# drprojects/superpoint_transformer

Hardware: AMD Instinct MI355X
Metric: Mpoints/s SPT fwd+bwd on S3DIS-scale NAG (higher is better)
Workload: dtype f32 (the reference's shipped matmul class - configs/train.yaml:60-61 `float32_matmul_precision: high` = TF32 / bf16x3 next to `precision: 32` - as bf16x3: matrix products on the bf16 pipe with split operands, attention and the backward of the fused layers and of the attention blocks' Linears hi*hi +

## Files before the change

include/spt_hip.h:

```cpp
#ifndef SPT_HIP_H
#define SPT_HIP_H

#include <stddef.h>
#include <stdint.h>

#ifdef __cplusplus
extern "C" {
#endif

typedef void* spt_stream_t;

enum spt_reduce_op {
  SPT_SUM = 0,
  SPT_MEAN = 1,
  SPT_MIN = 2,
  SPT_MAX = 3
};

typedef struct spt_gn_fwd_tables {
  const float* weight;
  const float* mean_scale;
  float eps;
  float* mean;
  float* rstd;
  float* am;
  float* scale;
} spt_gn_fwd_tables;
typedef struct spt_gn_bwd_tables {
  const float* weight;
  const float* mean_scale;
  const float* mean;
  const float* rstd;
  float* c1;
  float* c2;
  float* c3;
  float* gweight;
  float* gbias;
  float* gmean_scale;
} spt_gn_bwd_tables;

int spt_version(void);
const char* spt_last_error(void);

size_t spt_csr_build_workspace_bytes(int64_t n, int64_t num_seg);
int spt_csr_build(const int64_t* idx, int64_t n, int64_t num_seg,
                  int32_t* perm, int32_t* rowptr,
                  void* ws, size_t ws_bytes, spt_stream_t stream);
int spt_csr_pos_seg(const int32_t* rowptr, int64_t num_seg, int64_t n, int32_t* pos_seg,
                    spt_stream_t stream);
int spt_csr_gather_i64_i32(const int64_t* src, const int32_t* perm, int64_t n, int32_t* out,
                           spt_stream_t stream);

int spt_segcsr_reduce_f32(int op, const float* x, const int32_t* perm,
                          const int32_t* rowptr, int64_t n, int64_t num_seg,
                          int c, float* out, int32_t* arg, spt_stream_t stream);
int spt_segcsr_use_stream(int on);
int spt_segcsr_reduce_ex_f32(int op, const float* x, const int32_t* perm,
                             const int32_t* rowptr, int64_t n, int64_t num_seg,
                             int c, float* out, int32_t* arg, int formulation,
                             spt_stream_t stream);
int spt_segcsr_max_affine_ex_f32(const float* x, const int32_t* perm, const int32_t* rowptr,
                                 int64_t n, int64_t num_seg, int c, const float* am,
                                 const float* scale, const float* bias, float act_slope,
                                 const int64_t* seg_graph, float* out, int32_t* arg,
                                 int formulation, spt_stream_t stream);

int spt_segcsr_max_affine_f32(const float* x, const int32_t* perm, const int32_t* rowptr,
                              int64_t n, int64_t num_seg, int c, const float* am,
                              const float* scale, const float* bias, float act_slope,
                              const int64_t* seg_graph, float* out, int32_t* arg,
                              spt_stream_t stream);
int spt_segcsr_max_affine_bf16_supported(int c, int64_t n);
int spt_segcsr_max_affine_bf16(const void* x_bf16, const int32_t* perm, const int32_t* rowptr,
                               int64_t n, int64_t num_seg, int c, const float* am,
                               const float* scale, const float* bias, float act_slope,
                               const int64_t* seg_graph, float* out, int32_t* arg,
                               spt_stream_t stream);
int spt_segcsr_max_affine_raw_supported(int c, int64_t n);
int spt_segcsr_max_affine_raw_f32(const void* x, int x_is_bf16, const int32_t* perm,
                                  const int32_t* rowptr, int64_t n, int64_t num_seg, int c,
                                  const float* am, const float* scale, const float* bias,
                                  float act_slope, const int64_t* seg_graph, float* out,
                                  int32_t* arg, float* raw, spt_stream_t stream);
int spt_segcsr_reduce_bwd_f32(int op, const float* gout, const int32_t* arg,
                              const int64_t* idx, const int32_t* perm,
                              const int32_t* rowptr, int64_t n, int64_t num_seg,
                              int c, float* gx, spt_stream_t stream);


int spt_segcsr_sum_i64(const int64_t* x, const int32_t* perm,
                       const int32_t* rowptr, int64_t n, int64_t num_seg,
                       int c, int64_t* out, spt_stream_t stream);

int spt_gather_rows_f32(const float* x, const int64_t* idx, int64_t n,
                        int64_t num_src, int c, float* out, spt_stream_t stream);

int spt_unit_sphere_norm_f32(const float* pos, const int64_t* idx,
                             const int32_t* perm, const int32_t* rowptr,
                             const float* w_f32, const int64_t* w_i64,
                             int64_t n, int64_t num_seg, float* pos_out,
                             float* diam, float* center, spt_stream_t stream);
int spt_unit_sphere_assemble_f32(const float* pos, const int64_t* idx,
                                 const int32_t* perm, const int32_t* rowptr,
                                 const float* w_f32, const int64_t* w_i64,
                                 int64_t n, int64_t num_seg, const float* x, int cx,
                                 float* xcat, float* diam, float* center, spt_stream_t stream);
size_t spt_unit_sphere_workspace_bytes(int64_t n, int64_t num_seg);
int spt_unit_sphere_norm_ws_f32(const float* pos, const int64_t* idx, const int32_t* perm,
                                const int32_t* rowptr, const float* w_f32, const int64_t* w_i64,
                                int64_t n, int64_t num_seg, float* pos_out, float* diam,
                                float* center, void* ws, size_t ws_bytes, spt_stream_t stream);
int spt_unit_sphere_assemble_ws_f32(const float* pos, const int64_t* idx, const int32_t* perm,
                                    const int32_t* rowptr, const float* w_f32, const int64_t* w_i64,
                                    int64_t n, int64_t num_seg, const float* x, int cx, float* xcat,
                                    float* diam, float* center, void* ws, size_t ws_bytes,
                                    spt_stream_t stream);

size_t spt_graphnorm_workspace_bytes(int64_t r, int d, int num_graphs);
int spt_graphnorm_fwd_f32(const float* x, const int64_t* batch, int64_t r, int d,
                          int num_graphs, const float* weight, const float* bias,
                          const float* mean_scale, float eps, float act_slope,
                          float* y, float* mean, float* rstd, void* ws,
                          size_t ws_bytes, spt_stream_t stream);
int spt_graphnorm_bwd_f32(const float* x, const float* gy, const int64_t* batch,
                          int64_t r, int d, int num_graphs, const float* weight,
                          const float* bias, const float* mean_scale,
                          const float* mean, const float* rstd, float act_slope,
                          float* gx, float* gweight, float* gbias,
                          float* gmean_scale, void* ws, size_t ws_bytes,
                          spt_stream_t stream);
int spt_graphnorm_stats_f32(const float* x, const int64_t* batch, int64_t r, int d, int num_graphs,
                            const float* weight, const float* mean_scale, float eps, float* mean,
                            float* rstd, float* am, float* scale, void* ws, size_t ws_bytes,
                            spt_stream_t stream);
// ... 676 lines not shown
```

superpoint_transformer_amd/_lib.py:

```python
import ctypes
import os

import torch

_HERE = os.path.dirname(os.path.abspath(__file__))
LIB_PATH = os.path.join(_HERE, "lib", "libspt_hip.so")

_c = ctypes
_i64 = _c.c_int64
_int = _c.c_int
_p = _c.c_void_p
_sz = _c.c_size_t
_f32 = _c.c_float
_f64 = _c.c_double

SIGNATURES = {
    "spt_version": (_int, []),
    "spt_last_error": (_c.c_char_p, []),
    "spt_csr_build_workspace_bytes": (_sz, [_i64, _i64]),
    "spt_csr_build": (_int, [_p, _i64, _i64, _p, _p, _p, _sz, _p]),
    "spt_csr_pos_seg": (_int, [_p, _i64, _i64, _p, _p]),
    "spt_csr_gather_i64_i32": (_int, [_p, _p, _i64, _p, _p]),
    "spt_segcsr_reduce_f32": (_int, [_int, _p, _p, _p, _i64, _i64, _int, _p, _p, _p]),
    "spt_segcsr_max_affine_f32": (_int, [_p, _p, _p, _i64, _i64, _int, _p, _p, _p, _f32, _p, _p, _p, _p]),
    "spt_segcsr_max_affine_bf16_supported": (_int, [_int, _i64]),
    "spt_segcsr_max_affine_bf16": (_int, [_p, _p, _p, _i64, _i64, _int, _p, _p, _p, _f32, _p, _p, _p, _p]),
    "spt_segcsr_max_affine_raw_supported": (_int, [_int, _i64]),
    "spt_segcsr_max_affine_raw_f32": (_int, [_p, _int, _p, _p, _i64, _i64, _int, _p, _p, _p, _f32, _p, _p, _p,
                                             _p, _p]),
    "spt_graphnorm_bwd_stats_sparse_raw_f32": (_int, [_p, _p, _p, _p, _p, _i64, _i64, _int, _int, _p, _p, _p,
                                                      _f32, _p, _p, _sz, _p]),
    "spt_fused_linear_storage_supported": (_int, [_int, _int]),
    "spt_graphnorm_bwd_stats_sparse_ex_f32": (_int, [_p, _int, _p, _p, _p, _p, _i64, _i64, _int, _int, _p, _p,
                                                     _p, _f32, _p, _p, _sz, _p]),
    "spt_segcsr_reduce_bwd_f32": (_int, [_int, _p, _p, _p, _p, _p, _i64, _i64, _int, _p, _p]),
    "spt_segcsr_sum_i64": (_int, [_p, _p, _p, _i64, _i64, _int, _p, _p]),
    "spt_gather_rows_f32": (_int, [_p, _p, _i64, _i64, _int, _p, _p]),
    "spt_graphnorm_workspace_bytes": (_sz, [_i64, _int, _int]),
    "spt_graphnorm_fwd_f32": (_int, [_p, _p, _i64, _int, _int, _p, _p, _p, _f32, _f32,
                                     _p, _p, _p, _p, _sz, _p]),
    "spt_graphnorm_bwd_f32": (_int, [_p, _p, _p, _i64, _int, _int, _p, _p, _p, _p, _p,
                                     _f32, _p, _p, _p, _p, _p, _sz, _p]),
    "spt_graphnorm_stats_f32": (_int, [_p, _p, _i64, _int, _int, _p, _p, _f32, _p, _p, _p, _p,
                                       _p, _sz, _p]),
    "spt_graphnorm_bwd_acc_f32": (_int, [_p, _p, _p, _i64, _int, _int, _p, _p, _p, _p, _p,
                                         _f32, _p, _p, _p, _p, _p, _p, _sz, _p]),
    "spt_edge_attn_fwd_f32": (_int, [_p, _i64, _int, _int, _int, _p, _p, _p, _i64, _p, _int,
                                     _p, _p, _p, _p, _p, _p, _int, _f32, _p, _p, _p, _p]),
    "spt_edge_attn_bwd_workspace_bytes": (_sz, [_int, _int, _int, _int]),
    "spt_attn_use_mfma": (_int, [_int]),
    "spt_attn_bwd_packed": (_int, [_int]),
    "spt_attn_bwd_el_full_line": (_int, [_int]),
    "spt_attn_bwd_el_target_order": (_int, [_int]),
    "spt_attn_tile_record_ints": (_int, []),
    "spt_attn_pack_tile_ids_ex": (_int, [_p, _p, _p, _p, _i64, _p, _p]),
    "spt_attn_tile_record_ints_m": (_int, [_int]),
    "spt_attn_pack_tile_ids_m": (_int, [_p, _p, _p, _p, _i64, _int, _p, _p]),
    "spt_attn_mirror_prepare": (_int, [_p, _p, _i64, _i64, _p, _p, _p]),
    "spt_attn_pack_tile_ids_mirror": (_int, [_p, _p, _p, _p, _i64, _i64, _p, _p]),
    "spt_attn_split_pack_f32": (_int, [_p, _i64, _int, _int, _p, _p]),
    "spt_attn_split_grad_f32": (_int, [_p, _i64, _int, _int, _p, _p]),
    "spt_edge_attn_bwd_f32": (_int, [_p, _i64, _int, _int, _int, _p, _p, _p, _i64, _p, _int,
                                     _p, _p, _p, _p, _p, _p, _int, _f32, _p, _p, _p, _p,
                                     _p, _p, _p, _p, _p, _p, _p, _p, _p, _sz, _p]),
    "spt_edge_attn_bwd_acc_f32": (_int, [_p, _i64, _int, _int, _int, _p, _p, _p, _i64, _p, _int,
                                         _p, _p, _p, _p, _p, _p, _int, _f32, _p, _p, _p, _p,
                                         _p, _p, _int, _p, _p, _p, _p, _p, _p, _p, _sz, _p]),
    "spt_edge_attn_fwd_ex_f32": (_int, [_p, _i64, _int, _int, _int, _p, _p, _p, _i64, _p, _int,
                                        _p, _p, _p, _p, _p, _p, _int, _f32, _p, _p, _p, _int, _p]),
    "spt_attn_resolve_mode": (_int, [_int]),
    "spt_edge_attn_bwd_route": (_int, [_i64, _i64, _int, _int, _int, _int, _int, _int, _sz]),
    "spt_edge_attn_bwd_ex_workspace_bytes": (_sz, [_i64, _i64, _int, _int, _int, _int]),
    "spt_edge_attn_bwd_el_supported": (_int, [_int, _int, _int, _int, _int]),
    "spt_attn_pack_tile_ids": (_int, [_p, _p, _p, _i64, _p, _p]),
    "spt_edge_attn_bwd_ex_f32": (_int, [_p, _i64, _int, _int, _int, _p, _p, _p, _p, _p, _p, _p, _i64, _p, _int,
                                        _p, _p, _p, _p, _p, _p, _int, _f32, _p, _p, _p, _p,
                                        _p, _p, _int, _p, _p, _p, _p, _p, _p, _int, _p, _sz, _p]),
    "spt_grid_knn_workspace_bytes": (_sz, [_i64, _i64]),
    "spt_knn_use_cell_path": (_int, [_int]),
    "spt_segcsr_use_stream": (_int, [_int]),
    "spt_segcsr_reduce_ex_f32": (_int, [_int, _p, _p, _p, _i64, _i64, _int, _p, _p, _int, _p]),
    "spt_segcsr_max_affine_ex_f32": (_int, [_p, _p, _p, _i64, _i64, _int, _p, _p, _p, _f32, _p, _p, _p,
                                            _int, _p]),
    "spt_grid_knn_ex_f32": (_int, [_p, _i64, _p, _i64, _int, _f32, _f32, _p, _p, _int, _int, _int,
                                   _p, _p, _p, _int, _p, _sz, _p]),
    "spt_grid_knn_geof_f32": (_int, [_p, _i64, _int, _f32, _f32, _p, _p, _int, _int, _int, _int,
                                     _p, _p, _p, _p, _int, _p, _sz, _p]),
    "spt_grid_knn_after_f32": (_int, [_p, _i64, _p, _i64, _int, _f32, _f32, _p, _p, _int, _int, _p, _p,
                                      _p, _p, _p, _sz, _p]),
    "spt_grid_knn_f32": (_int, [_p, _i64, _p, _i64, _int, _f32, _f32, _p, _p, _int, _int, _int,
                                _p, _p, _p, _p, _sz, _p]),
    "spt_point_geof_dense_f32": (_int, [_p, _i64, _p, _int, _int, _int, _int, _p, _p, _p]),
    "spt_point_geof_dense_ld_f32": (_int, [_p, _i64, _p, _int, _i64, _int, _int, _int, _p, _p, _p]),
    "spt_bbox_f32": (_int, [_p, _i64, _p, _p]),
    "spt_knn_subsample_f32": (_int, [_p, _i64, _p, _f32, _int, _p, _p, _p]),
    "spt_grid_cell_ids_f32": (_int, [_p, _i64, _f32, _p, _p, _p, _p]),
    "spt_grid_count_cells_workspace_bytes": (_sz, [_i64]),
    "spt_grid_count_cells_f32": (_int, [_p, _i64, _f32, _p, _p, _p, _p, _sz, _p]),
    "spt_spatial_order_workspace_bytes": (_sz, [_i64, _i64]),
    "spt_spatial_order": (_int, [_p, _i64, _f32, _p, _p, _p, _p, _sz, _p]),
    "spt_point_geof_csr_f32": (_int, [_p, _i64, _p, _p, _int, _int, _int, _p, _p]),
    "spt_vertical_edge_features_f32": (_int, [_p, _i64] + [_p] * 13 + [_p]),
    "spt_edge_affinity_features_f32": (_int, [_p, _i64, _int, _p, _p, _i64, _p, _p]),
    "spt_edge_affinity_features_bwd_f32": (_int, [_p, _p, _i64, _int, _p, _p, _i64, _p, _p]),
    "spt_scatter_pca_f32": (_int, [_p, _p, _p, _i64, _p, _p, _p]),
# ... 271 lines not shown
```

superpoint_transformer_amd/csr.py:

```python
import weakref

import torch

from . import _lib

_ATTR = "_spt_csr_memo"
_ATTR_BAD = "_spt_csr_rejected"


class SegmentCSR:

    __slots__ = ("idx", "perm", "rowptr", "n", "num_seg", "_pos_seg")

    def __init__(self, idx, perm, rowptr, n, num_seg):
        self.idx = idx
        self.perm = perm
        self.rowptr = rowptr
        self.n = n
        self.num_seg = num_seg
        self._pos_seg = None

    def pos_seg(self):
        if self._pos_seg is None:
            out = torch.empty(max(self.n, 1), dtype=torch.int32, device=self.perm.device)
            with torch.cuda.device(out.device):
                st = _lib.lib.spt_csr_pos_seg(_lib.ptr(self.rowptr), self.num_seg, self.n,
                                              _lib.ptr(out), _lib.stream_ptr(out.device))
            _lib.check(st, "spt_csr_pos_seg")
            self._pos_seg = out[:self.n]
        return self._pos_seg

    def counts(self):
        return (self.rowptr[1:] - self.rowptr[:-1])


def build_csr(idx, num_seg):
    _lib.require_cuda(idx)
    if idx.dim() != 1:
        raise ValueError("segment index must be 1-D")
    idx = _lib.dense(idx, torch.int64, 8)
    n = idx.numel()
    num_seg = int(num_seg)
    if num_seg < 1:
        num_seg = 1
    dev = idx.device
    perm = torch.empty(max(n, 1), dtype=torch.int32, device=dev)
    rowptr = torch.empty(num_seg + 1, dtype=torch.int32, device=dev)
    ws_bytes = _lib.lib.spt_csr_build_workspace_bytes(n, num_seg)
    ws = torch.empty(max(ws_bytes, 1), dtype=torch.uint8, device=dev)
    with torch.cuda.device(dev):
        st = _lib.lib.spt_csr_build(
            _lib.ptr(idx), n, num_seg, _lib.ptr(perm), _lib.ptr(rowptr),
            _lib.ptr(ws), ws_bytes, _lib.stream_ptr(dev))
    _lib.check(st, "spt_csr_build")
    return SegmentCSR(idx.detach(), perm[:n], rowptr, n, num_seg)


def csr_of(idx, num_seg=None):
    if isinstance(idx, SegmentCSR):
        return idx
    if num_seg is None:
        num_seg = int(idx.max().item()) + 1 if idx.numel() > 0 else 1
    num_seg = max(int(num_seg), 1)
    memo = getattr(idx, _ATTR, None)
    key = (idx._version, num_seg, idx.data_ptr(), idx.numel())
    if memo is not None and key in memo:
        return memo[key]
    csr = build_csr(idx, num_seg)
    if memo is None or any(k[0] != idx._version for k in memo):
        memo = {}
        try:
            setattr(idx, _ATTR, memo)
        except Exception:
            return csr
    memo[key] = csr
    return csr


_USE_SUB_VIEWS = True
_USE_MIRROR = True


def use_mirror_views(on=True):
    global _USE_MIRROR
    old, _USE_MIRROR = _USE_MIRROR, bool(on)
    return old


def use_sub_views(on=True):
    global _USE_SUB_VIEWS
    old, _USE_SUB_VIEWS = _USE_SUB_VIEWS, bool(on)
    return old


class StaleCSRError(RuntimeError):
    """A stored ``sub`` adopted as the CSR view of a ``super_index`` turned out not to describe it."""


_PENDING = []
_CHECK_BITS = {1: "pointers do not run 0 .. n monotonically", 2: "a point id outside [0, n)",
               4: "membership: idx[points[j]] is not the cluster holding position j",
               8: "the points of a cluster are not in ascending order"}
_ORDER_ONLY = 8
_PINNED = {}


def _flag_text(v):
    return "; ".join(t for b, t in _CHECK_BITS.items() if v & b) or "ok"


def _pinned_slot():
    ring = _PINNED.get("ring")
    if ring is None:
        ring = _PINNED["ring"] = torch.zeros(256, dtype=torch.int32).pin_memory()
        _PINNED["next"] = 0
    busy = {h.data_ptr() for ev, h, *_ in _PENDING if ev is not None}
    for _ in range(ring.numel()):
        i = _PINNED["next"]
        _PINNED["next"] = (i + 1) % ring.numel()
        slot = ring[i:i + 1]
        if slot.data_ptr() not in busy:
            return slot
    return torch.zeros(1, dtype=torch.int32).pin_memory()


_MIRROR_BITS = {1: "a pair (i, i + M) that is not (s, t) / (t, s)", 2: "a self loop with s != t"}
MIRROR_ATTR = "_spt_mirror_pairs"


def _drop_view(ref, key, vkey, remember):
    idx = ref() if ref is not None else None
    if idx is None:
        return
    memo = getattr(idx, _ATTR, None)
    if memo is not None:
        memo.pop(key, None)
    if remember:
        try:
            setattr(idx, _ATTR_BAD, vkey)
        except Exception:
            pass


def verify_adopted(block=False):
    keep, failed = [], None
    for item in _PENDING:
        ev, host, what, ref, key, vkey = item
        if ev is None:
            if not block:
                keep.append(item)
                continue
            v = int(host.item())
        else:
            if block:
                ev.synchronize()
            if not ev.query():
                keep.append(item)
                continue
            v = int(host[0])
        if v and key == "mirror":
            ei = ref() if ref is not None else None
            if ei is not None:
                for a in (MIRROR_ATTR, _ATTR):
# ... 8 lines not shown
        if v:
            _drop_view(ref, key, vkey, remember=True)
        if v & ~_ORDER_ONLY and failed is None:
            failed = (what, v, None)
    _PENDING[:] = keep
    if failed is not None and failed[2] is not None:
        raise StaleCSRError(
            f"{failed[0]} was declared [i<j | j>i | loops] with mirrored halves ({MIRROR_ATTR}) but is not "
            f"({failed[2]}): the attention backward of that batch paired wrong edges - drop the attribute "
            "or rebuild the edge list (the hint has been removed: later batches sort by target)")
    if failed is not None:
        raise StaleCSRError(
            f"the stored CSR adopted as the view of {failed[0]} does not describe it "
            f"({_flag_text(failed[1])}): the segment kernels grouped wrong rows since that batch (inside "
            "their buffers: the adopted view is clamped) - rebuild the NAG's `sub` or call "
            "csr.use_sub_views(False)")


def adopt_csr(idx, num_seg, pointers, points, ascending=None, verify="now"):
    if not _USE_SUB_VIEWS or idx is None or ascending is False:
        return None
    n = idx.numel()
    num_seg = max(int(num_seg), 1)
    if (points.numel() != n or pointers.numel() != num_seg + 1
            or points.device != idx.device or pointers.device != idx.device):
        return None
    if idx.dtype != torch.int64 or not idx.is_contiguous() or idx.dim() != 1:
        return None
    _lib.require_cuda(idx)
    capturing = torch.cuda.is_current_stream_capturing()
    if _PENDING and not capturing:
        verify_adopted()
    memo = getattr(idx, _ATTR, None)
    key = (idx._version, num_seg, idx.data_ptr(), n)
    if memo is not None and key in memo:
        return memo[key]
    bad = getattr(idx, _ATTR_BAD, None)
    vkey = key + (points.data_ptr(), points._version, pointers.data_ptr(), pointers._version)
    if bad == vkey:
        return None
    dev = idx.device
    pl, ql = _lib.dense(points, torch.int64, 8), _lib.dense(pointers, torch.int64, 8)
    flag = torch.zeros(1, dtype=torch.int32, device=dev)
    perm = torch.empty(max(n, 1), dtype=torch.int32, device=dev)
    rowptr = torch.empty(num_seg + 1, dtype=torch.int32, device=dev)
    with torch.cuda.device(dev):
        st = _lib.lib.spt_csr_adopt_i64(_lib.ptr(idx), _lib.ptr(pl), _lib.ptr(ql), n, num_seg,
                                        _lib.ptr(perm), _lib.ptr(rowptr), _lib.ptr(flag),
                                        _lib.stream_ptr(dev))
    _lib.check(st, "spt_csr_adopt_i64")
    what = f"an index of {n} rows / {num_seg} segments"
    try:
        ref = weakref.ref(idx)
    except TypeError:
        ref = None
    if verify == "deferred" and capturing:
        _PENDING.append((None, flag, what, ref, key, vkey))
    elif verify == "deferred":
        host = _pinned_slot()
        host.copy_(flag, non_blocking=True)
        ev = torch.cuda.Event()
        ev.record(torch.cuda.current_stream(dev))
        _PENDING.append((ev, host, what, ref, key, vkey))
    elif int(flag.item()):
        try:
            setattr(idx, _ATTR_BAD, vkey)
        except Exception:
            pass
        return None
    csr = SegmentCSR(idx.detach(), perm[:n], rowptr, n, num_seg)
    if memo is None or any(k[0] != idx._version for k in memo):
        memo = {}
        try:
            setattr(idx, _ATTR, memo)
        except Exception:
            return csr
    memo[key] = csr
    return csr


class EdgeCSR:

    __slots__ = ("erowptr", "eperm", "tgt_sorted", "n", "e", "_view", "_src_sorted", "_tview",
                 "_tile_ids", "_ei", "_mirror", "_ei_ref")

    def __init__(self, erowptr, eperm, tgt_sorted, n, e, view=None, edge_index=None):
        self.erowptr, self.eperm, self.tgt_sorted, self.n, self.e = \
            erowptr, eperm, tgt_sorted, n, e
        self._view = view
        self._src_sorted = None
        self._tview = None
        self._tile_ids = None
        self._ei = self._mirror = self._ei_ref = None
        m = getattr(edge_index, MIRROR_ATTR, None) if edge_index is not None else None
        if (_USE_MIRROR and m is not None and edge_index._version == 0 and edge_index.dtype == torch.int64
                and edge_index.is_contiguous() and edge_index.dim() == 2 and 0 <= 2 * int(m) <= e):
            self._ei, self._mirror = edge_index.detach(), int(m)
            try:
                self._ei_ref = weakref.ref(edge_index)
            except TypeError:
                pass

    def mirrored(self, mode=-1):
        return self._mirror is not None and int(_lib.lib.spt_attn_tile_record_ints_m(int(mode))) == 64

    def tile_ids(self, mode=-1):
        ints = int(_lib.lib.spt_attn_tile_record_ints_m(int(mode)))
        if self._tile_ids is None:
            self._tile_ids = {}
        if ints not in self._tile_ids:
            dev = self.tgt_sorted.device
            nt = (self.e + 15) // 16
            out = torch.empty((max(nt, 1), ints), dtype=torch.int32, device=dev)
            src = self.src_sorted()
            if ints == 64 and self._mirror is not None:
                self._pack_mirror(out, src, dev)
                self._tile_ids[ints] = out
                return out
            tperm = self.target_view().perm if ints == 64 else None
            order = (1 << 6) if ints == 64 else (2 << 6)
            with torch.cuda.device(dev):
                st = _lib.lib.spt_attn_pack_tile_ids_m(
                    _lib.ptr(self.eperm), _lib.ptr(self.tgt_sorted), _lib.ptr(src), _lib.ptr(tperm),
                    self.e, order, _lib.ptr(out), _lib.stream_ptr(dev))
            _lib.check(st, "spt_attn_pack_tile_ids_m")
            self._tile_ids[ints] = out
        return self._tile_ids[ints]

    def _pack_mirror(self, out, src, dev):
        inv = torch.empty(max(self.e, 1), dtype=torch.int32, device=dev)
        flag = torch.zeros(1, dtype=torch.int32, device=dev)
        sp = _lib.stream_ptr(dev)
        with torch.cuda.device(dev):
            st = _lib.lib.spt_attn_mirror_prepare(_lib.ptr(self._ei), _lib.ptr(self.eperm), self.e,
                                                  self._mirror, _lib.ptr(inv), _lib.ptr(flag), sp)
            _lib.check(st, "spt_attn_mirror_prepare")
            st = _lib.lib.spt_attn_pack_tile_ids_mirror(
                _lib.ptr(self.eperm), _lib.ptr(self.tgt_sorted), _lib.ptr(src), _lib.ptr(inv), self.e,
                self._mirror, _lib.ptr(out), sp)
            _lib.check(st, "spt_attn_pack_tile_ids_mirror")
        what = f"an edge list of {self.e} edges ({self._mirror} pairs)"
        if torch.cuda.is_current_stream_capturing():
            _PENDING.append((None, flag, what, self._ei_ref, "mirror", None))
        else:
            host = _pinned_slot()
            host.copy_(flag, non_blocking=True)
            ev = torch.cuda.Event()
            ev.record(torch.cuda.current_stream(dev))
            _PENDING.append((ev, host, what, self._ei_ref, "mirror", None))

    def target_view(self):
        if self._tview is None:
            self._tview = build_csr(self.tgt_sorted.long(), self.n)
        return self._tview

    def src_sorted(self):
        if self._src_sorted is None:
            if self._view is not None:
                self._src_sorted = self._view.pos_seg()
            else:
                cnt = (self.erowptr[1:] - self.erowptr[:-1]).long()
                self._src_sorted = torch.repeat_interleave(
                    torch.arange(self.n, device=cnt.device, dtype=torch.int32), cnt)
        return self._src_sorted


def edge_csr_of(edge_index, num_nodes):
    if isinstance(edge_index, EdgeCSR):
        return edge_index
    memo = getattr(edge_index, _ATTR, None)
    key = (edge_index._version, int(num_nodes), edge_index.data_ptr(), edge_index.shape[1])
    if memo is not None and key in memo:
        return memo[key]
    view = build_csr(edge_index[0], num_nodes)
    e = edge_index.shape[1]
    tgt_sorted = torch.empty(max(e, 1), dtype=torch.int32, device=edge_index.device)[:e]
    tgt64 = _lib.dense(edge_index[1], torch.int64, 8)
    with torch.cuda.device(edge_index.device):
        st = _lib.lib.spt_csr_gather_i64_i32(_lib.ptr(tgt64), _lib.ptr(view.perm), e,
                                             _lib.ptr(tgt_sorted), _lib.stream_ptr(edge_index.device))
    _lib.check(st, "spt_csr_gather_i64_i32")
    if _PENDING and not torch.cuda.is_current_stream_capturing():
        verify_adopted()
    ecsr = EdgeCSR(view.rowptr, view.perm, tgt_sorted, int(num_nodes), edge_index.shape[1], view,
                   edge_index=edge_index)
    if memo is None or any(k[0] != edge_index._version for k in memo):
        memo = {}
        try:
            setattr(edge_index, _ATTR, memo)
        except Exception:
            return ecsr
    memo[key] = ecsr
    return ecsr


def forget(*tensors):
    for t in tensors:
        if t is None:
            continue
        for a in (_ATTR, _ATTR_BAD, "_spt_graph_runs", "_spt_graph_runs_via", "_spt_graph_ranges",
                  "_spt_batch_checked"):
            if hasattr(t, a):
                try:
                    delattr(t, a)
                except Exception:
                    pass
```

superpoint_transformer_amd/csrc/csr_build.hip:

```cpp
#include "radix_sort.hpp"

using namespace spt;

extern "C" size_t spt_csr_build_workspace_bytes(int64_t n, int64_t num_seg) {
  if (n < 0 || num_seg < 1) return 0;
  return RadixScratch::bytes(n);
}

extern "C" int spt_csr_build(const int64_t* idx, int64_t n, int64_t num_seg,
                             int32_t* perm, int32_t* rowptr, void* ws,
                             size_t ws_bytes, spt_stream_t stream_) {
  hipStream_t stream = (hipStream_t)stream_;
  SPT_CHECK_ARG(n >= 0 && n < ((int64_t)1 << 31) - SORT_TILE, "n out of range");
  SPT_CHECK_ARG(num_seg >= 1 && num_seg < ((int64_t)1 << 31), "num_seg out of range");
  SPT_CHECK_ARG(rowptr != nullptr, "rowptr is null");
  SPT_CHECK_ARG(n == 0 || (idx && perm), "null idx/perm");
  const size_t need = RadixScratch::bytes(n);
  SPT_CHECK_ARG(ws_bytes >= need && (ws || need == 0), "workspace too small");

  if (n == 0) {
    rowptr_from_sorted_kernel<<<stream_grid(num_seg + 1, 256), 256, 0, stream>>>(
        nullptr, 0, num_seg, rowptr);
    SPT_CHECK_LAUNCH();
    return 0;
  }
  if (num_seg <= 1) {
    iota_kernel<<<stream_grid(n, 256), 256, 0, stream>>>(perm, n);
    rowptr_single_kernel<<<1, 1, 0, stream>>>(rowptr, n);
    SPT_CHECK_LAUNCH();
    return 0;
  }
  RadixScratch s;
  s.carve((char*)ws, n);
  const uint32_t *ks, *vs;
  SPT_CHECK_ARG(radix_sort_pairs<1>(idx, nullptr, nullptr, n, bits_for(num_seg), s,
                                    (uint32_t*)perm, &ks, &vs, stream) == 0,
                "scan partials do not fit their region");
  rowptr_from_sorted_kernel<<<stream_grid(n + 1, 256), 256, 0, stream>>>(
      ks, n, num_seg, rowptr);
  SPT_CHECK_LAUNCH();
  return 0;
}


namespace spt {
__global__ __launch_bounds__(256) void csr_pos_seg_kernel(const int32_t* __restrict__ rowptr,
                                                          int64_t num_seg,
                                                          int32_t* __restrict__ pos_seg) {
  const int sub = threadIdx.x & 15;
  const int64_t stride = (int64_t)gridDim.x * 16;
  for (int64_t s = (int64_t)blockIdx.x * 16 + (threadIdx.x >> 4); s < num_seg; s += stride) {
    const int a = rowptr[s], b = rowptr[s + 1];
    for (int j = a + sub; j < b; j += 16) pos_seg[j] = (int32_t)s;
  }
}
__global__ __launch_bounds__(256) void csr_gather_i64_i32_kernel(const int64_t* __restrict__ src,
                                                                 const int32_t* __restrict__ perm,
                                                                 int64_t n, int32_t* __restrict__ out) {
  const int64_t stride = (int64_t)gridDim.x * blockDim.x;
  for (int64_t j = (int64_t)blockIdx.x * blockDim.x + threadIdx.x; j < n; j += stride)
    out[j] = (int32_t)src[perm[j]];
}
}

extern "C" int spt_csr_pos_seg(const int32_t* rowptr, int64_t num_seg, int64_t n, int32_t* pos_seg,
                               spt_stream_t stream_) {
  hipStream_t stream = (hipStream_t)stream_;
  SPT_CHECK_ARG(num_seg >= 0 && n >= 0, "bad shape");
  if (n == 0 || num_seg == 0) return 0;
  SPT_CHECK_ARG(rowptr && pos_seg, "null pointer");
  spt::csr_pos_seg_kernel<<<spt::stream_grid(num_seg, 16), 256, 0, stream>>>(rowptr, num_seg, pos_seg);
  SPT_CHECK_LAUNCH();
  return 0;
}

extern "C" int spt_csr_gather_i64_i32(const int64_t* src, const int32_t* perm, int64_t n,
                                      int32_t* out, spt_stream_t stream_) {
  hipStream_t stream = (hipStream_t)stream_;
  SPT_CHECK_ARG(n >= 0, "bad shape");
  if (n == 0) return 0;
  SPT_CHECK_ARG(src && perm && out, "null pointer");
  spt::csr_gather_i64_i32_kernel<<<spt::stream_grid(n, 256), 256, 0, stream>>>(src, perm, n, out);
  SPT_CHECK_LAUNCH();
  return 0;
}
```

superpoint_transformer_amd/csrc/radix_sort.hpp:

```cpp
#pragma once
#include "common.hpp"

namespace spt {


constexpr int SORT_THREADS = 256;
constexpr int SORT_WAVES = SORT_THREADS / 64;
constexpr int SORT_ITEMS = 16;
constexpr int SORT_TILE = SORT_THREADS * SORT_ITEMS;
constexpr int WAVE_CHUNK = SORT_TILE / SORT_WAVES;
constexpr int MAX_BINS = 256;

template <int MODE>
__device__ __forceinline__ uint32_t load_key(const int64_t* __restrict__ idx,
                                             const uint32_t* __restrict__ keys,
                                             int64_t i) {
  if constexpr (MODE == 1)
    return (uint32_t)idx[i];
  else
    return keys[i];
}

template <int MODE>
__global__ __launch_bounds__(SORT_THREADS) void radix_hist_kernel(
// ... 223 lines not shown
  while (((int64_t)1 << b) < num_seg) ++b;
  return b;
}

struct RadixScratch {
  uint32_t *k0, *k1, *v0, *v1, *hist, *part;
  int64_t part_cap;
  static size_t bytes(int64_t n) {
    const int64_t m = n > 0 ? n : 1;
    const int nblocks = (int)ceil_div(m, SORT_TILE);
    const int64_t hist_len = (int64_t)MAX_BINS * nblocks;
    return 4 * align_up((size_t)m * 4, 256) + align_up((size_t)hist_len * 4, 256) +
           scan_part_bytes(hist_len);
  }
  char* carve(char* base, int64_t n) {
    const int64_t m = n > 0 ? n : 1;
    const size_t nb = align_up((size_t)m * 4, 256);
    const int nblocks = (int)ceil_div(m, SORT_TILE);
    const int64_t hist_len = (int64_t)MAX_BINS * nblocks;
    k0 = (uint32_t*)base; base += nb;
    k1 = (uint32_t*)base; base += nb;
    v0 = (uint32_t*)base; base += nb;
    v1 = (uint32_t*)base; base += nb;
    hist = (uint32_t*)base; base += align_up((size_t)hist_len * 4, 256);
    part = (uint32_t*)base; base += scan_part_bytes(hist_len);
    part_cap = (int64_t)(scan_part_bytes(hist_len) / 4);
    return base;
  }
};

static inline int device_exclusive_scan(uint32_t* data, int64_t m, uint32_t* part,
                                        int64_t part_cap, hipStream_t stream) {
  if (scan_part_entries(m) > part_cap) return -1;
  const int nch = (int)scan_part_entries(m);
  scan_reduce_kernel<<<nch, SCAN_THREADS, 0, stream>>>(data, m, part);
  scan_partials_kernel<<<1, SCAN_THREADS, 0, stream>>>(part, nch);
  scan_apply_kernel<<<nch, SCAN_THREADS, 0, stream>>>(data, m, part);
  return 0;
}

template <int MODE>
static inline int radix_sort_pairs(const int64_t* idx64, const uint32_t* keys32,
                                    const uint32_t* vals32, int64_t n, int nbits,
                                    RadixScratch& s, uint32_t* final_vals,
                                    const uint32_t** keys_sorted,
                                    const uint32_t** vals_sorted, hipStream_t stream) {
  const int nblocks = (int)ceil_div(n, SORT_TILE);
  const int passes = (nbits + 7) / 8;
  const int per = (nbits + passes - 1) / passes;
  if (scan_part_entries((int64_t)(1 << per) * nblocks) > s.part_cap) return -1;
  uint32_t* kbuf[2] = {s.k0, s.k1};
  uint32_t* vbuf[2] = {s.v0, s.v1};
  const uint32_t* kin = keys32;
  const uint32_t* vin = vals32;
  int shift = 0;
  for (int pass = 0; pass < passes; ++pass) {
    const int bits = (nbits - shift < per) ? (nbits - shift) : per;
    uint32_t* kout = kbuf[pass & 1];
    uint32_t* vout = vbuf[pass & 1];
    if (pass == passes - 1 && final_vals) vout = final_vals;
    const int64_t hl = (int64_t)(1 << bits) * nblocks;
    if (pass == 0) {
      radix_hist_kernel<MODE><<<nblocks, SORT_THREADS, 0, stream>>>(
          idx64, kin, n, shift, bits, s.hist, nblocks);
      if (device_exclusive_scan(s.hist, hl, s.part, s.part_cap, stream)) return -1;
      radix_scatter_kernel<MODE><<<nblocks, SORT_THREADS, 0, stream>>>(
          idx64, kin, vin, n, shift, bits, s.hist, nblocks, kout, vout);
    } else {
      radix_hist_kernel<0><<<nblocks, SORT_THREADS, 0, stream>>>(
          nullptr, kin, n, shift, bits, s.hist, nblocks);
      if (device_exclusive_scan(s.hist, hl, s.part, s.part_cap, stream)) return -1;
      radix_scatter_kernel<0><<<nblocks, SORT_THREADS, 0, stream>>>(
          nullptr, kin, vin, n, shift, bits, s.hist, nblocks, kout, vout);
    }
    kin = kout;
    vin = vout;
    shift += bits;
  }
  *keys_sorted = kin;
  *vals_sorted = vin;
  return 0;
}

}
```

Measured before the change: 371.6.

## Fuse edge CSR build into one radix sort carrying targets, inverse and mirror check

```diff
diff --git a/include/spt_hip.h b/include/spt_hip.h
--- a/include/spt_hip.h
+++ b/include/spt_hip.h
@@ -50,6 +50,11 @@
                     spt_stream_t stream);
 int spt_csr_gather_i64_i32(const int64_t* src, const int32_t* perm, int64_t n, int32_t* out,
                            spt_stream_t stream);
+size_t spt_edge_csr_build_workspace_bytes(int64_t e, int64_t n);
+int spt_edge_csr_build(const int64_t* edge_index, int64_t e, int64_t n, int64_t pairs,
+                       int32_t* erowptr, int32_t* eperm, int32_t* tgt_sorted, int32_t* src_sorted,
+                       int32_t* inv, int32_t* tile_ids, int32_t* flag, void* ws, size_t ws_bytes,
+                       spt_stream_t stream);
 
 int spt_segcsr_reduce_f32(int op, const float* x, const int32_t* perm,
                           const int32_t* rowptr, int64_t n, int64_t num_seg,
diff --git a/superpoint_transformer_amd/_lib.py b/superpoint_transformer_amd/_lib.py
--- a/superpoint_transformer_amd/_lib.py
+++ b/superpoint_transformer_amd/_lib.py
@@ -21,6 +21,8 @@
     "spt_csr_build": (_int, [_p, _i64, _i64, _p, _p, _p, _sz, _p]),
     "spt_csr_pos_seg": (_int, [_p, _i64, _i64, _p, _p]),
     "spt_csr_gather_i64_i32": (_int, [_p, _p, _i64, _p, _p]),
+    "spt_edge_csr_build_workspace_bytes": (_sz, [_i64, _i64]),
+    "spt_edge_csr_build": (_int, [_p, _i64, _i64, _i64, _p, _p, _p, _p, _p, _p, _p, _p, _sz, _p]),
     "spt_segcsr_reduce_f32": (_int, [_int, _p, _p, _p, _i64, _i64, _int, _p, _p, _p]),
     "spt_segcsr_max_affine_f32": (_int, [_p, _p, _p, _i64, _i64, _int, _p, _p, _p, _f32, _p, _p, _p, _p]),
     "spt_segcsr_max_affine_bf16_supported": (_int, [_int, _i64]),
diff --git a/superpoint_transformer_amd/csr.py b/superpoint_transformer_amd/csr.py
--- a/superpoint_transformer_amd/csr.py
+++ b/superpoint_transformer_amd/csr.py
@@ -1,3 +1,4 @@
+import os
 import weakref
 
 import torch
@@ -79,6 +80,13 @@
 
 _USE_SUB_VIEWS = True
 _USE_MIRROR = True
+_USE_FUSED_EDGE = os.environ.get("SPT_EDGE_CSR_FUSED", "1") != "0"
+
+
+def use_fused_edge_build(on=True):
+    global _USE_FUSED_EDGE
+    old, _USE_FUSED_EDGE = _USE_FUSED_EDGE, bool(on)
+    return old
 
 
 def use_mirror_views(on=True):
@@ -253,7 +261,7 @@
 class EdgeCSR:
 
     __slots__ = ("erowptr", "eperm", "tgt_sorted", "n", "e", "_view", "_src_sorted", "_tview",
-                 "_tile_ids", "_ei", "_mirror", "_ei_ref")
+                 "_tile_ids", "_ei", "_mirror", "_ei_ref", "_inv", "_flag")
 
     def __init__(self, erowptr, eperm, tgt_sorted, n, e, view=None, edge_index=None):
         self.erowptr, self.eperm, self.tgt_sorted, self.n, self.e = \
@@ -263,6 +271,7 @@
         self._tview = None
         self._tile_ids = None
         self._ei = self._mirror = self._ei_ref = None
+        self._inv = self._flag = None
         m = getattr(edge_index, MIRROR_ATTR, None) if edge_index is not None else None
         if (_USE_MIRROR and m is not None and edge_index._version == 0 and edge_index.dtype == torch.int64
                 and edge_index.is_contiguous() and edge_index.dim() == 2 and 0 <= 2 * int(m) <= e):
@@ -310,6 +319,11 @@
                 _lib.ptr(self.eperm), _lib.ptr(self.tgt_sorted), _lib.ptr(src), _lib.ptr(inv), self.e,
                 self._mirror, _lib.ptr(out), sp)
             _lib.check(st, "spt_attn_pack_tile_ids_mirror")
+        self._inv = inv[:self.e]
+        self._defer_mirror_verdict(flag, dev)
+
+    def _defer_mirror_verdict(self, flag, dev):
+        self._flag = flag
         what = f"an edge list of {self.e} edges ({self._mirror} pairs)"
         if torch.cuda.is_current_stream_capturing():
             _PENDING.append((None, flag, what, self._ei_ref, "mirror", None))
@@ -343,6 +357,9 @@
     key = (edge_index._version, int(num_nodes), edge_index.data_ptr(), edge_index.shape[1])
     if memo is not None and key in memo:
         return memo[key]
+    if _USE_FUSED_EDGE and edge_index.dim() == 2 and edge_index.shape[1] > 0:
+        ecsr = _edge_csr_fused(edge_index, num_nodes)
+        return _memoise_edge(edge_index, memo, key, ecsr)
     view = build_csr(edge_index[0], num_nodes)
     e = edge_index.shape[1]
     tgt_sorted = torch.empty(max(e, 1), dtype=torch.int32, device=edge_index.device)[:e]
@@ -355,6 +372,10 @@
         verify_adopted()
     ecsr = EdgeCSR(view.rowptr, view.perm, tgt_sorted, int(num_nodes), edge_index.shape[1], view,
                    edge_index=edge_index)
+    return _memoise_edge(edge_index, memo, key, ecsr)
+
+
+def _memoise_edge(edge_index, memo, key, ecsr):
     if memo is None or any(k[0] != edge_index._version for k in memo):
         memo = {}
         try:
@@ -362,6 +383,37 @@
         except Exception:
             return ecsr
     memo[key] = ecsr
+    return ecsr
+
+
+def _edge_csr_fused(edge_index, num_nodes):
+    _lib.require_cuda(edge_index)
+    dev = edge_index.device
+    e, n = edge_index.shape[1], max(int(num_nodes), 1)
+    ei = _lib.dense(edge_index, torch.int64, 8)
+    i32 = dict(dtype=torch.int32, device=dev)
+    erowptr = torch.empty(n + 1, **i32)
+    eperm, tgt_sorted, src_sorted = (torch.empty(e, **i32) for _ in range(3))
+    if _PENDING and not torch.cuda.is_current_stream_capturing():
+        verify_adopted()
+    ecsr = EdgeCSR(erowptr, eperm, tgt_sorted, int(num_nodes), e, None, edge_index=edge_index)
+    records = ecsr._mirror is not None and int(_lib.lib.spt_attn_tile_record_ints_m(-1)) == 64
+    inv = torch.empty(e, **i32) if records else None
+    ids = torch.empty(((e + 15) // 16, 64), **i32) if records else None
+    flag = torch.empty(1, **i32)
+    ws_bytes = _lib.lib.spt_edge_csr_build_workspace_bytes(e, n)
+    ws = torch.empty(max(ws_bytes, 1), dtype=torch.uint8, device=dev)
+    with torch.cuda.device(dev):
+        st = _lib.lib.spt_edge_csr_build(
+            _lib.ptr(ei), e, n, ecsr._mirror if records else -1, _lib.ptr(erowptr), _lib.ptr(eperm),
+            _lib.ptr(tgt_sorted), _lib.ptr(src_sorted), _lib.ptr(inv), _lib.ptr(ids), _lib.ptr(flag),
+            _lib.ptr(ws), ws_bytes, _lib.stream_ptr(dev))
+    _lib.check(st, "spt_edge_csr_build")
+    ecsr._src_sorted = src_sorted
+    if records:
+        ecsr._inv = inv
+        ecsr._tile_ids = {64: ids}
+        ecsr._defer_mirror_verdict(flag, dev)
     return ecsr
 
 
diff --git a/superpoint_transformer_amd/csrc/csr_build.hip b/superpoint_transformer_amd/csrc/csr_build.hip
--- a/superpoint_transformer_amd/csrc/csr_build.hip
+++ b/superpoint_transformer_amd/csrc/csr_build.hip
@@ -84,3 +84,103 @@
   SPT_CHECK_LAUNCH();
   return 0;
 }
+
+
+#include "edge_attn_internal.hpp"
+
+namespace spt {
+struct EdgeCsrPlan {
+  int nblocks;
+  size_t off_k[2], off_v[2], off_t[2], off_hist, off_tot, off_bad, total;
+};
+static inline EdgeCsrPlan edge_csr_plan(int64_t e) {
+  EdgeCsrPlan p;
+  const int64_t m = e > 0 ? e : 1;
+  p.nblocks = (int)ceil_div(m, SORT_TILE);
+  const size_t nb = align_up((size_t)m * 4, 256);
+  size_t o = 0;
+  for (int i = 0; i < 2; ++i) {
+    p.off_k[i] = o; o += nb;
+    p.off_v[i] = o; o += nb;
+    p.off_t[i] = o; o += nb;
+  }
+  p.off_hist = o; o += align_up((size_t)MAX_BINS * p.nblocks * 4, 256);
+  p.off_tot = o;  o += align_up((size_t)MAX_BINS * 4, 256);
+  p.off_bad = o;  o += align_up((size_t)p.nblocks * 4, 256);
+  p.total = o;
+  return p;
+}
+}
+
+extern "C" size_t spt_edge_csr_build_workspace_bytes(int64_t e, int64_t n) {
+  if (e < 0 || n < 1) return 0;
+  return spt::edge_csr_plan(e).total;
+}
+
+extern "C" int spt_edge_csr_build(const int64_t* edge_index, int64_t e, int64_t n, int64_t pairs,
+                                  int32_t* erowptr, int32_t* eperm, int32_t* tgt_sorted,
+                                  int32_t* src_sorted, int32_t* inv, int32_t* tile_ids,
+                                  int32_t* flag, void* ws, size_t ws_bytes, spt_stream_t stream_) {
+  hipStream_t stream = (hipStream_t)stream_;
+  SPT_CHECK_ARG(e >= 1 && e < ((int64_t)1 << 31) - SORT_TILE, "e out of range");
+  SPT_CHECK_ARG(n >= 1 && n < ((int64_t)1 << 31), "n out of range");
+  SPT_CHECK_ARG(pairs >= -1 && 2 * pairs <= e, "bad mirror count");
+  SPT_CHECK_ARG(edge_index && erowptr && eperm && tgt_sorted && src_sorted && flag, "null pointer");
+  SPT_CHECK_ARG(pairs >= 0 || !tile_ids, "tile records need a mirror count");
+  SPT_CHECK_ARG(!tile_ids || inv, "tile records need inv");
+  const EdgeCsrPlan p = edge_csr_plan(e);
+  SPT_CHECK_ARG(ws && ws_bytes >= p.total, "workspace too small");
+  char* w = (char*)ws;
+  uint32_t* kbuf[2] = {(uint32_t*)(w + p.off_k[0]), (uint32_t*)(w + p.off_k[1])};
+  uint32_t* vbuf[2] = {(uint32_t*)(w + p.off_v[0]), (uint32_t*)(w + p.off_v[1])};
+  int32_t* tbuf[2] = {(int32_t*)(w + p.off_t[0]), (int32_t*)(w + p.off_t[1])};
+  uint32_t* hist = (uint32_t*)(w + p.off_hist);
+  uint32_t* tot = (uint32_t*)(w + p.off_tot);
+  uint32_t* bad = (uint32_t*)(w + p.off_bad);
+
+  const int nbits = bits_for(n);
+  const int passes = (nbits + 7) / 8;
+  const int per = (nbits + passes - 1) / passes;
+  const int nblocks = p.nblocks;
+  const uint32_t* kin = nullptr;
+  const uint32_t* vin = nullptr;
+  const int32_t* tin = nullptr;
+  int shift = 0;
+  for (int pass = 0; pass < passes; ++pass) {
+    const int bits = (nbits - shift < per) ? (nbits - shift) : per;
+    const bool last = pass == passes - 1;
+    uint32_t* kout = last ? (uint32_t*)src_sorted : kbuf[pass & 1];
+    uint32_t* vout = last ? (uint32_t*)eperm : vbuf[pass & 1];
+    int32_t* tout = last ? tgt_sorted : tbuf[pass & 1];
+    if (pass == 0)
+      edge_hist_kernel<true><<<nblocks, SORT_THREADS, 0, stream>>>(
+          edge_index, nullptr, e, shift, bits, hist, nblocks, pairs, bad);
+    else
+      edge_hist_kernel<false><<<nblocks, SORT_THREADS, 0, stream>>>(
+          nullptr, kin, e, shift, bits, hist, nblocks, -1, nullptr);
+    edge_rowscan_kernel<<<1 << bits, SCAN_THREADS, 0, stream>>>(hist, nblocks, tot, bad,
+                                                               pass == 0 ? flag : nullptr);
+    if (pass == 0 && last)
+      edge_scatter_kernel<1, true><<<nblocks, SORT_THREADS, 0, stream>>>(
+          edge_index, nullptr, nullptr, nullptr, e, shift, bits, hist, tot, nblocks, kout, vout, tout, inv);
+    else if (pass == 0)
+      edge_scatter_kernel<1, false><<<nblocks, SORT_THREADS, 0, stream>>>(
+          edge_index, nullptr, nullptr, nullptr, e, shift, bits, hist, tot, nblocks, kout, vout, tout, nullptr);
+    else if (last)
+      edge_scatter_kernel<0, true><<<nblocks, SORT_THREADS, 0, stream>>>(
+          nullptr, kin, vin, tin, e, shift, bits, hist, tot, nblocks, kout, vout, tout, inv);
+    else
+      edge_scatter_kernel<0, false><<<nblocks, SORT_THREADS, 0, stream>>>(
+          nullptr, kin, vin, tin, e, shift, bits, hist, tot, nblocks, kout, vout, tout, nullptr);
+    kin = kout;
+    vin = vout;
+    tin = tout;
+    shift += bits;
+  }
+  rowptr_from_sorted_kernel<<<stream_grid(e + 1, 256), 256, 0, stream>>>(
+      (const uint32_t*)src_sorted, e, n, erowptr);
+  if (tile_ids)
+    attn_pack_tile_ids_mirror_launch(eperm, tgt_sorted, src_sorted, inv, e, pairs, tile_ids, stream);
+  SPT_CHECK_LAUNCH();
+  return 0;
+}
diff --git a/superpoint_transformer_amd/csrc/radix_sort.hpp b/superpoint_transformer_amd/csrc/radix_sort.hpp
--- a/superpoint_transformer_amd/csrc/radix_sort.hpp
+++ b/superpoint_transformer_amd/csrc/radix_sort.hpp
@@ -329,4 +329,188 @@
   return 0;
 }
 
-}
+
+template <bool FIRST>
+__global__ __launch_bounds__(SORT_THREADS) void edge_hist_kernel(
+    const int64_t* __restrict__ ei, const uint32_t* __restrict__ keys_in, int64_t n, int shift,
+    int bits, uint32_t* __restrict__ blockhist, int nblocks, int64_t pairs,
+    uint32_t* __restrict__ blockbad) {
+  __shared__ uint32_t h[MAX_BINS];
+  __shared__ uint32_t sbad;
+  h[threadIdx.x] = 0;
+  if (threadIdx.x == 0) sbad = 0;
+  __syncthreads();
+  const int64_t base = (int64_t)blockIdx.x * SORT_TILE;
+  const uint32_t mask = (1u << bits) - 1u;
+  uint32_t bad = 0;
+#pragma unroll
+  for (int k = 0; k < SORT_ITEMS; ++k) {
+    const int64_t i = base + (int64_t)k * SORT_THREADS + threadIdx.x;
+    if (i < n) {
+      uint32_t key;
+      if constexpr (FIRST) {
+        const int64_t s = ei[i];
+        key = (uint32_t)s;
+        if (pairs >= 0) {
+          const int64_t t = ei[n + i];
+          if (i < pairs) {
+            if (ei[i + pairs] != t || ei[n + i + pairs] != s) bad |= 1u;
+          } else if (i >= 2 * pairs) {
+            if (s != t) bad |= 2u;
+          }
+        }
+      } else {
+        key = keys_in[i];
+      }
+      atomicAdd(&h[(key >> shift) & mask], 1u);
+    }
+  }
+  if constexpr (FIRST)
+    if (bad) atomicOr(&sbad, bad);
+  __syncthreads();
+  if ((int)threadIdx.x < (1 << bits))
+    blockhist[(size_t)threadIdx.x * nblocks + blockIdx.x] = h[threadIdx.x];
+  if constexpr (FIRST)
+    if (threadIdx.x == 0) blockbad[blockIdx.x] = sbad;
+}
+
+static __global__ __launch_bounds__(SCAN_THREADS) void edge_rowscan_kernel(
+    uint32_t* __restrict__ blockhist, int nblocks, uint32_t* __restrict__ digit_total,
+    const uint32_t* __restrict__ blockbad, int32_t* __restrict__ flag) {
+  uint32_t* row = blockhist + (size_t)blockIdx.x * nblocks;
+  uint32_t carry = 0;
+  for (int base = 0; base < nblocks; base += SCAN_THREADS) {
+    const int i = base + threadIdx.x;
+    const uint32_t v = (i < nblocks) ? row[i] : 0u;
+    uint32_t tot;
+    const uint32_t ex = block_exclusive_scan(v, &tot);
+    if (i < nblocks) row[i] = carry + ex;
+    carry += tot;
+  }
+  if (threadIdx.x == 0) digit_total[blockIdx.x] = carry;
+  if (blockIdx.x == 0 && flag) {
+    __shared__ uint32_t sbad;
+    if (threadIdx.x == 0) sbad = 0;
+    __syncthreads();
+    uint32_t bad = 0;
+    for (int i = threadIdx.x; i < nblocks; i += SCAN_THREADS) bad |= blockbad[i];
+    if (bad) atomicOr(&sbad, bad);
+    __syncthreads();
+    if (threadIdx.x == 0) *flag = (int32_t)sbad;
+  }
+}
+
+template <int MODE, bool LAST>
+__global__ __launch_bounds__(SORT_THREADS) void edge_scatter_kernel(
+    const int64_t* __restrict__ ei, const uint32_t* __restrict__ keys_in,
+    const uint32_t* __restrict__ vals_in, const int32_t* __restrict__ tgts_in, int64_t n, int shift,
+    int bits, const uint32_t* __restrict__ blockoff, const uint32_t* __restrict__ digit_total,
+    int nblocks, uint32_t* __restrict__ keys_out, uint32_t* __restrict__ vals_out,
+    int32_t* __restrict__ tgts_out, int32_t* __restrict__ inv) {
+  __shared__ uint32_t buf[3 * SORT_TILE];
+  __shared__ uint32_t dbase[MAX_BINS];
+  __shared__ uint32_t texcl[MAX_BINS];
+  static_assert(SORT_WAVES * MAX_BINS <= 3 * SORT_TILE && MAX_BINS == SORT_THREADS, "LDS plan");
+  uint32_t(*cnt)[MAX_BINS] = reinterpret_cast<uint32_t(*)[MAX_BINS]>(buf);
+  const int w = threadIdx.x >> 6;
+  const int lane = threadIdx.x & 63;
+  const int bins = 1 << bits;
+  const bool own = (int)threadIdx.x < bins;
+  for (int j = threadIdx.x; j < SORT_WAVES * MAX_BINS; j += SORT_THREADS) buf[j] = 0;
+
+  const int64_t tbase = (int64_t)blockIdx.x * SORT_TILE;
+  const int64_t wbase = tbase + (int64_t)w * WAVE_CHUNK;
+  const uint32_t mask = (uint32_t)bins - 1u;
+  const uint64_t lt = lanemask_lt();
+
+  uint32_t key[SORT_ITEMS];
+  uint32_t val[SORT_ITEMS];
+  int32_t tgt[SORT_ITEMS];
+  uint32_t rank[SORT_ITEMS];
+#pragma unroll
+  for (int r = 0; r < SORT_ITEMS; ++r) {
+    const int64_t i = wbase + r * 64 + lane;
+    const bool valid = i < n;
+    if constexpr (MODE == 1) {
+      key[r] = valid ? (uint32_t)ei[i] : 0xffffffffu;
+      val[r] = (uint32_t)i;
+      tgt[r] = valid ? (int32_t)ei[n + i] : 0;
+    } else {
+      key[r] = valid ? keys_in[i] : 0xffffffffu;
+      val[r] = valid ? vals_in[i] : 0u;
+      tgt[r] = valid ? tgts_in[i] : 0;
+    }
+  }
+  {
+    const uint32_t t = own ? digit_total[threadIdx.x] : 0u;
+    const uint32_t ex = block_exclusive_scan(t, nullptr);
+    if (own) dbase[threadIdx.x] = ex;
+  }
+  __syncthreads();
+#pragma unroll
+  for (int r = 0; r < SORT_ITEMS; ++r) {
+    const int64_t i = wbase + r * 64 + lane;
+    const bool valid = i < n;
+    const uint32_t d = (key[r] >> shift) & mask;
+    uint64_t peers = __ballot(valid);
+    for (int b = 0; b < bits; ++b) {
+      const bool bit = (d >> b) & 1u;
+      const uint64_t m = __ballot(valid && bit);
+      peers &= bit ? m : ~m;
+    }
+    const uint32_t pre = cnt[w][d];
+    const uint32_t rk = __popcll(peers & lt);
+    const uint32_t tot = __popcll(peers);
+    rank[r] = pre + rk;
+    __builtin_amdgcn_wave_barrier();
+    if (valid && rk == tot - 1) cnt[w][d] = pre + tot;
+    __builtin_amdgcn_wave_barrier();
+  }
+  __syncthreads();
+  {
+    uint32_t tc = 0;
+    if (own) {
+#pragma unroll
+      for (int w2 = 0; w2 < SORT_WAVES; ++w2) {
+        const uint32_t t = cnt[w2][threadIdx.x];
+        cnt[w2][threadIdx.x] = tc;
+        tc += t;
+      }
+    }
+    const uint32_t ex = block_exclusive_scan(tc, nullptr);
+    if (own) {
+      texcl[threadIdx.x] = ex;
+      dbase[threadIdx.x] += blockoff[(size_t)threadIdx.x * nblocks + blockIdx.x] - ex;
+    }
+  }
+  __syncthreads();
+#pragma unroll
+  for (int r = 0; r < SORT_ITEMS; ++r) {
+    const uint32_t d = (key[r] >> shift) & mask;
+    rank[r] += texcl[d] + cnt[w][d];
+  }
+  __syncthreads();
+#pragma unroll
+  for (int r = 0; r < SORT_ITEMS; ++r) {
+    const int64_t i = wbase + r * 64 + lane;
+    if (i < n) {
+      buf[rank[r]] = key[r];
+      buf[SORT_TILE + rank[r]] = val[r];
+      buf[2 * SORT_TILE + rank[r]] = (uint32_t)tgt[r];
+    }
+  }
+  __syncthreads();
+  const int tn = (int)((n - tbase) < (int64_t)SORT_TILE ? (n - tbase) : (int64_t)SORT_TILE);
+  for (int j = threadIdx.x; j < tn; j += SORT_THREADS) {
+    const uint32_t k = buf[j];
+    const uint32_t v = buf[SORT_TILE + j];
+    const uint32_t dst = dbase[(k >> shift) & mask] + (uint32_t)j;
+    keys_out[dst] = k;
+    vals_out[dst] = v;
+    tgts_out[dst] = (int32_t)buf[2 * SORT_TILE + j];
+    if constexpr (LAST)
+      if (inv) inv[v] = (int32_t)dst;
+  }
+}
+
+}
```

After: 377.2 (median of 6 runs). +1.5%, better.
